# tusen-ai/SST

Hardware: AMD Instinct MI355X
Metric: LiDAR frames/sec (SST backbone fwd+bwd) at Waymo 0.32m voxels (higher is better)
Workload: dtype f32 (storage, accumulation, attention, LayerNorm, reductions: fp32; the dense products of the encoder layers from the EXACT three-way bf16 split of both fp32 operands, six bf16 MFMA products with fp32 accumulation - error vs float64 <= 2 x the fp32 matrix pipe's: tests/test_gpu_dense_f32x6.py)

## Files before the change

### sst_amd/csrc/layer_tail_x6.hip

```cpp
#include <math.h>
#include <stdlib.h>
#include "common.h"

#ifndef SST_NT_OUT
#define SST_NT_OUT false
#endif
#ifndef SST_NT_BWD
#define SST_NT_BWD true
#endif

namespace {

typedef float f32x4 __attribute__((ext_vector_type(4)));
typedef float f32x2 __attribute__((ext_vector_type(2)));
typedef unsigned u32x4 __attribute__((ext_vector_type(4)));
typedef __bf16 bf16x8 __attribute__((ext_vector_type(8)));
typedef __bf16 bf16x2 __attribute__((ext_vector_type(2)));

__device__ __forceinline__ unsigned pack2(float lo, float hi) {
  const f32x2 v = {lo, hi};
  return __builtin_bit_cast(unsigned, __builtin_convertvector(v, bf16x2));
}
__device__ __forceinline__ float lo_f(unsigned p) { return __uint_as_float(p << 16); }
__device__ __forceinline__ float hi_f(unsigned p) { return __uint_as_float(p & 0xffff0000u); }
__device__ __forceinline__ f32x4 mma32(u32x4 a, u32x4 b, f32x4 c) {
  return __builtin_amdgcn_mfma_f32_16x16x32_bf16(__builtin_bit_cast(bf16x8, a), __builtin_bit_cast(bf16x8, b), c, 0, 0, 0);
}
__device__ __forceinline__ void split2(float a, float b, unsigned& p0, unsigned& p1, unsigned& p2) {
  p0 = pack2(a, b);
  const float ra = a - lo_f(p0), rb = b - hi_f(p0);
  p1 = pack2(ra, rb);
  p2 = pack2(ra - lo_f(p1), rb - hi_f(p1));
}
struct img3 {
  u32x4 p0, p1, p2;
};
__device__ __forceinline__ img3 split8(const f32x4& a, const f32x4& b) {
  unsigned q0[4], q1[4], q2[4];
  split2(a[0], a[1], q0[0], q1[0], q2[0]);
  split2(a[2], a[3], q0[1], q1[1], q2[1]);
  split2(b[0], b[1], q0[2], q1[2], q2[2]);
  split2(b[2], b[3], q0[3], q1[3], q2[3]);
  img3 r;
  r.p0 = (u32x4){q0[0], q0[1], q0[2], q0[3]};
  r.p1 = (u32x4){q1[0], q1[1], q1[2], q1[3]};
  r.p2 = (u32x4){q2[0], q2[1], q2[2], q2[3]};
  return r;
}
__device__ __forceinline__ void join8(const img3& v, f32x4& a, f32x4& b) {
#pragma unroll
  for (int i = 0; i < 2; ++i) {
    a[2 * i] = (lo_f(v.p2[i]) + lo_f(v.p1[i])) + lo_f(v.p0[i]);
    a[2 * i + 1] = (hi_f(v.p2[i]) + hi_f(v.p1[i])) + hi_f(v.p0[i]);
    b[2 * i] = (lo_f(v.p2[2 + i]) + lo_f(v.p1[2 + i])) + lo_f(v.p0[2 + i]);
    b[2 * i + 1] = (hi_f(v.p2[2 + i]) + hi_f(v.p1[2 + i])) + hi_f(v.p0[2 + i]);
  }
}

__device__ __forceinline__ float erf_as(float z, float& e) {
  const float az = fabsf(z);
  const float t = __builtin_amdgcn_rcpf(fmaf(0.3275911f, az, 1.f));
  e = __expf(-az * az);
  const float poly = t * fmaf(t, fmaf(t, fmaf(t, fmaf(t, 1.061405429f, -1.453152027f), 1.421413741f), -0.284496736f), 0.254829592f);
  return copysignf(fmaf(-poly, e, 1.f), z);
}
__device__ __forceinline__ float gelu_f(float x) {
  float e;
  return 0.5f * x * (1.f + erf_as(x * 0.70710678118654752f, e));
}
__device__ __forceinline__ float gelu_grad_f(float x) {
  float e;
  const float phi = 0.5f * (1.f + erf_as(x * 0.70710678118654752f, e));
  return fmaf(x * 0.3989422804014327f, e, phi);
}

__device__ __forceinline__ int w_lds_row(int n) {
  const int tp = n >> 5, within = n & 31;
  return 16 * (2 * tp + ((within >> 2) & 1)) + ((within >> 3) << 2) + (within & 3);
}

template <int CTRL>
__device__ __forceinline__ float dpp_add(float v) {
  return v + __int_as_float(__builtin_amdgcn_update_dpp(0, __float_as_int(v), CTRL, 0xf, 0xf, false));
}
__device__ __forceinline__ float row_sum16(float v) {
  v = dpp_add<0xB1>(v);
  v = dpp_add<0x4E>(v);
  v = dpp_add<0x141>(v);
  return dpp_add<0x140>(v);
}

constexpr int kC = 128, kFF = 256, kHC = 32, kNF = kFF / kHC;
constexpr int kFrag = 1024;
constexpr int kI1 = 2 * 4 * kFrag;
constexpr int kI2 = 8 * 1 * kFrag;
constexpr int kIA = 8 * 2 * kFrag;
constexpr int kPart1 = 3 * kI1, kPart2 = 3 * kI2;
constexpr int kSlot = kPart1 + kPart2;
static_assert(3 * kIA <= kSlot, "slot");
#ifndef SST_TAIL_WAVES
#define SST_TAIL_WAVES 4
#endif
constexpr int kWaves = SST_TAIL_WAVES, kNTH = 64 * kWaves, kRowsPerWg = 16 * kWaves;
static_assert(kNTH >= 2 * kC, "one thread per LayerNorm parameter-gradient column");
constexpr int kNChunks = kNF + 2;
constexpr int kPackDir = kNChunks * kSlot;
constexpr int kParF = 6 * kC + kFF;
constexpr int kArea = kSlot;
constexpr int kScr = 2048;
constexpr int kLdsFwd = kArea + kParF * 4 + kWaves * kScr;
constexpr int kLdsBwd = kArea + 2 * kC * 4 + kWaves * 2 * kC * 4 + kWaves * kScr;

struct tail_weights {
  const float* wo;
  const float* w1;
  const float* w2;
};

template <bool BWD>
__device__ __forceinline__ void stage_load(const tail_weights W, int chunk, int t, float (&r)[16]) {
  if (!BWD) {
    if (chunk < 2) {
#pragma unroll
      for (int u = 0; u < 2; ++u) {
        const int idx = t + 512 * u, n = idx >> 3, k8 = (idx & 7) * 8;
        const float* p = W.wo + n * kC + 64 * chunk + k8;
        const f32x4 a = *(const f32x4*)p, b = *(const f32x4*)(p + 4);
#pragma unroll
        for (int e = 0; e < 4; ++e) r[8 * u + e] = a[e], r[8 * u + 4 + e] = b[e];
      }
    } else {
      const int j = chunk - 2;
      {
        const float* p = W.w1 + (size_t)(kHC * j + (t >> 4)) * kC + (t & 15) * 8;
        const f32x4 a = *(const f32x4*)p, b = *(const f32x4*)(p + 4);
#pragma unroll
        for (int e = 0; e < 4; ++e) r[e] = a[e], r[4 + e] = b[e];
      }
      {
        const float* p = W.w2 + (size_t)(t >> 2) * kFF + kHC * j + (t & 3) * 8;
        const f32x4 a = *(const f32x4*)p, b = *(const f32x4*)(p + 4);
#pragma unroll
        for (int e = 0; e < 4; ++e) r[8 + e] = a[e], r[12 + e] = b[e];
      }
    }
  } else {
    if (chunk >= kNF) {
      const int q = chunk - kNF;
#pragma unroll
      for (int u = 0; u < 2; ++u) {
        const int idx = t + 512 * u, jn = idx & 127, k8 = (idx >> 7) * 8;
        const float* p = W.wo + (size_t)(64 * q + k8) * kC + jn;
#pragma unroll
        for (int e = 0; e < 8; ++e) r[8 * u + e] = p[e * kC];
      }
    } else {
      const int j = chunk;
      {
        const float* p = W.w2 + (size_t)((t >> 5) * 8) * kFF + kHC * j + (t & 31);
#pragma unroll
        for (int e = 0; e < 8; ++e) r[e] = p[e * kFF];
      }
      {
        const float* p = W.w1 + (size_t)(kHC * j + (t >> 7) * 8) * kC + (t & 127);
#pragma unroll
        for (int e = 0; e < 8; ++e) r[8 + e] = p[e * kC];
      }
    }
  }
}

__device__ __forceinline__ int frag_off(int lr, int k8, int ks) {
  return ((lr >> 4) * ks + (k8 >> 5)) * kFrag + (16 * ((k8 >> 3) & 3) + (lr & 15)) * 16;
}

__device__ __forceinline__ void store_images(unsigned char* base, int image_bytes, int off, const float* v) {
  const f32x4 a = {v[0], v[1], v[2], v[3]}, b = {v[4], v[5], v[6], v[7]};
  const img3 s = split8(a, b);
  *(u32x4*)(base + off) = s.p0;
  *(u32x4*)(base + image_bytes + off) = s.p1;
  *(u32x4*)(base + 2 * image_bytes + off) = s.p2;
}

template <bool BWD>
__device__ __forceinline__ void stage_store(unsigned char* slot, int chunk, int t, const float (&r)[16]) {
  const bool outproj = BWD ? chunk >= kNF : chunk < 2;
  if (outproj) {
#pragma unroll
    for (int u = 0; u < 2; ++u) {
      const int idx = t + 512 * u;
      const int n = BWD ? (idx & 127) : (idx >> 3), k8 = BWD ? (idx >> 7) * 8 : (idx & 7) * 8;
      store_images(slot, kIA, frag_off(w_lds_row(n), k8, 2), r + 8 * u);
    }
  } else {
    const int n1 = BWD ? (t & 31) : (t >> 4), k1 = BWD ? (t >> 5) * 8 : (t & 15) * 8;
    store_images(slot, kI1, frag_off(w_lds_row(n1), k1, 4), r);
    const int n2 = BWD ? (t & 127) : (t >> 2), k2 = BWD ? (t >> 7) * 8 : (t & 3) * 8;
    store_images(slot + kPart1, kI2, frag_off(w_lds_row(n2), k2, 1), r + 8);
  }
}

constexpr int kPackMany = 16;
struct pack_batch {
  tail_weights w[kPackMany];
  unsigned char* dst[kPackMany];
};
__global__ __launch_bounds__(512) void encoder_tail_pack_k(const pack_batch B) {
  extern __shared__ __attribute__((aligned(16))) unsigned char lds[];
  const int layer = blockIdx.x / (2 * kNChunks), blk = blockIdx.x % (2 * kNChunks);
  const tail_weights W = B.w[layer];
  const int chunk = blk % kNChunks, dir = blk / kNChunks;
  float r[16];
  if (dir == 0) {
    stage_load<false>(W, chunk, threadIdx.x, r);
    stage_store<false>(lds, chunk, threadIdx.x, r);
  } else {
    stage_load<true>(W, chunk, threadIdx.x, r);
    stage_store<true>(lds, chunk, threadIdx.x, r);
  }
  __syncthreads();
  unsigned char* dst = B.dst[layer] + (size_t)blk * kSlot;
  for (int i = threadIdx.x; i < kSlot / 16; i += 512) *(u32x4*)(dst + 16 * i) = *(const u32x4*)(lds + 16 * i);
}

__device__ __forceinline__ void dma_pieces(const unsigned char* __restrict__ src, unsigned char* dst, int pieces, int wave, int lane) {
  for (int i = wave; i < pieces; i += kWaves)
    __builtin_amdgcn_global_load_lds((const __attribute__((address_space(1))) void*)(src + i * 1024 + lane * 16),
                                     (__attribute__((address_space(3))) void*)(dst + i * 1024), 16, 0, 0);
}

__device__ __forceinline__ void barrier_lds_only() { asm volatile("s_waitcnt lgkmcnt(0)\n\ts_barrier" ::: "memory"); }
__device__ __forceinline__ void barrier_drain() { asm volatile("s_waitcnt vmcnt(0) lgkmcnt(0)\n\ts_barrier" ::: "memory"); }

struct tile_io {
  unsigned char* scr;
  int frag_off0;
  int row_off[2];
  int64_t rrow[2];
  bool rvalid[2];
  int rcol;
};
__device__ __forceinline__ tile_io make_tile_io(unsigned char* scr, int lane, int64_t r0, int64_t m) {
  tile_io t;
  const int c = lane & 15, g = lane >> 4;
  t.scr = scr;
  t.frag_off0 = c * 128 + (((2 * g) ^ (c & 7)) << 4);
#pragma unroll
  for (int i = 0; i < 2; ++i) {
    const int r = 8 * i + (lane >> 3), p = lane & 7;
    t.row_off[i] = r * 128 + ((p ^ (r & 7)) << 4);
    t.rvalid[i] = r0 + r < m;
    t.rrow[i] = t.rvalid[i] ? r0 + r : m - 1;
  }
  t.rcol = (lane & 7) * 4;
  return t;
}
template <bool STREAM>
__device__ __forceinline__ void store32(const tile_io& t, float* __restrict__ base, int64_t ld, int col0, const f32x4& v0,
                                        const f32x4& v1) {
  *(f32x4*)(t.scr + t.frag_off0) = v0;
  *(f32x4*)(t.scr + (t.frag_off0 ^ 16)) = v1;
#pragma unroll
  for (int i = 0; i < 2; ++i) {
    const f32x4 w = *(const f32x4*)(t.scr + t.row_off[i]);
    if (t.rvalid[i]) {
      if (STREAM)
        __builtin_nontemporal_store(w, (f32x4*)(base + t.rrow[i] * ld + col0 + t.rcol));
      else
        *(f32x4*)(base + t.rrow[i] * ld + col0 + t.rcol) = w;
    }
  }
}
__device__ __forceinline__ void load32_issue(const tile_io& t, const float* __restrict__ base, int64_t ld, int col0, f32x4 (&w)[2]) {
#pragma unroll
  for (int i = 0; i < 2; ++i) w[i] = *(const f32x4*)(base + t.rrow[i] * ld + col0 + t.rcol);
}
__device__ __forceinline__ void load32_finish(const tile_io& t, const f32x4 (&w)[2], f32x4& v0, f32x4& v1) {
#pragma unroll
  for (int i = 0; i < 2; ++i) *(f32x4*)(t.scr + t.row_off[i]) = w[i];
  v0 = *(const f32x4*)(t.scr + t.frag_off0);
  v1 = *(const f32x4*)(t.scr + (t.frag_off0 ^ 16));
}

template <int HALF>
__device__ __forceinline__ void mma_half(const unsigned char* slot, int lane_off, const f32x4 (&x)[4][2], f32x4 (&acc)[8]) {
#pragma unroll
  for (int s2 = 0; s2 < 2; ++s2) {
    const img3 xs = split8(x[2 * HALF + s2][0], x[2 * HALF + s2][1]);
#pragma unroll
    for (int t0 = 0; t0 < 8; t0 += 4) {
      u32x4 a0[4], a1[4], a2[4];
#pragma unroll
      for (int u = 0; u < 4; ++u) {
        const int off = lane_off + ((t0 + u) * 2 + s2) * kFrag;
        a0[u] = *(const u32x4*)(slot + off);
        a1[u] = *(const u32x4*)(slot + kIA + off);
        a2[u] = *(const u32x4*)(slot + 2 * kIA + off);
      }
#pragma unroll
      for (int u = 0; u < 4; ++u) acc[t0 + u] = mma32(a0[u], xs.p2, acc[t0 + u]);
#pragma unroll
      for (int u = 0; u < 4; ++u) acc[t0 + u] = mma32(a2[u], xs.p0, acc[t0 + u]);
#pragma unroll
      for (int u = 0; u < 4; ++u) acc[t0 + u] = mma32(a1[u], xs.p1, acc[t0 + u]);
#pragma unroll
      for (int u = 0; u < 4; ++u) acc[t0 + u] = mma32(a0[u], xs.p1, acc[t0 + u]);
#pragma unroll
      for (int u = 0; u < 4; ++u) acc[t0 + u] = mma32(a1[u], xs.p0, acc[t0 + u]);
#pragma unroll
      for (int u = 0; u < 4; ++u) acc[t0 + u] = mma32(a0[u], xs.p0, acc[t0 + u]);
    }
  }
}

__device__ __forceinline__ void mma_first(const unsigned char* slot, int lane_off1, const img3 (&y)[4], f32x4& out0, f32x4& out1) {
  const f32x4 z = {0.f, 0.f, 0.f, 0.f};
  f32x4 am[2] = {z, z}, ca[2] = {z, z}, cb[2] = {z, z};
#pragma unroll
  for (int s = 0; s < 4; ++s) {
    u32x4 a0[2], a1[2], a2[2];
#pragma unroll
    for (int T = 0; T < 2; ++T) {
      const int off = lane_off1 + (T * 4 + s) * kFrag;
      a0[T] = *(const u32x4*)(slot + off);
      a1[T] = *(const u32x4*)(slot + kI1 + off);
      a2[T] = *(const u32x4*)(slot + 2 * kI1 + off);
    }
#pragma unroll
    for (int T = 0; T < 2; ++T) ca[T] = mma32(a0[T], y[s].p2, ca[T]);
#pragma unroll
    for (int T = 0; T < 2; ++T) cb[T] = mma32(a0[T], y[s].p1, cb[T]);
#pragma unroll
    for (int T = 0; T < 2; ++T) ca[T] = mma32(a2[T], y[s].p0, ca[T]);
#pragma unroll
    for (int T = 0; T < 2; ++T) am[T] = mma32(a0[T], y[s].p0, am[T]);
#pragma unroll
    for (int T = 0; T < 2; ++T) ca[T] = mma32(a1[T], y[s].p1, ca[T]);
#pragma unroll
    for (int T = 0; T < 2; ++T) cb[T] = mma32(a1[T], y[s].p0, cb[T]);
  }
  out0 = am[0] + (cb[0] + ca[0]);
  out1 = am[1] + (cb[1] + ca[1]);
}

__device__ __forceinline__ void mma_second(const unsigned char* slot2, int lane_off2, const img3& h, f32x4 (&acc)[8]) {
#pragma unroll
  for (int t0 = 0; t0 < 8; t0 += 4) {
    u32x4 a0[4], a1[4], a2[4];
#pragma unroll
    for (int u = 0; u < 4; ++u) {
      const int off = lane_off2 + (t0 + u) * kFrag;
      a0[u] = *(const u32x4*)(slot2 + off);
      a1[u] = *(const u32x4*)(slot2 + kI2 + off);
      a2[u] = *(const u32x4*)(slot2 + 2 * kI2 + off);
    }
#pragma unroll
    for (int u = 0; u < 4; ++u) acc[t0 + u] = mma32(a0[u], h.p2, acc[t0 + u]);
#pragma unroll
    for (int u = 0; u < 4; ++u) acc[t0 + u] = mma32(a2[u], h.p0, acc[t0 + u]);
#pragma unroll
    for (int u = 0; u < 4; ++u) acc[t0 + u] = mma32(a1[u], h.p1, acc[t0 + u]);
#pragma unroll
    for (int u = 0; u < 4; ++u) acc[t0 + u] = mma32(a0[u], h.p1, acc[t0 + u]);
#pragma unroll
    for (int u = 0; u < 4; ++u) acc[t0 + u] = mma32(a1[u], h.p0, acc[t0 + u]);
#pragma unroll
    for (int u = 0; u < 4; ++u) acc[t0 + u] = mma32(a0[u], h.p0, acc[t0 + u]);
  }
}

__device__ __forceinline__ void ln_stats(f32x4 (&v)[4][2], float eps, float& mean, float& rstd) {
  float sum = 0.f;
#pragma unroll
  for (int s = 0; s < 4; ++s)
#pragma unroll
    for (int r = 0; r < 4; ++r) sum += v[s][0][r] + v[s][1][r];
  sum += __shfl_xor(sum, 16, 64);
  sum += __shfl_xor(sum, 32, 64);
  mean = sum * (1.f / 128.f);
  float sq = 0.f;
#pragma unroll
  for (int s = 0; s < 4; ++s)
#pragma unroll
    for (int h = 0; h < 2; ++h)
#pragma unroll
      for (int r = 0; r < 4; ++r) {
        v[s][h][r] -= mean;
        sq = fmaf(v[s][h][r], v[s][h][r], sq);
      }
  sq += __shfl_xor(sq, 16, 64);
  sq += __shfl_xor(sq, 32, 64);
  rstd = rsqrtf(sq * (1.f / 128.f) + eps);
}

struct tail_fwd_params {
  const float *o, *x;
  const unsigned char* packed;
  const float *b_out, *b1, *b2, *n1w, *n1b, *n2w, *n2b;
  float eps;
  int64_t m;
  float *s1, *st1, *y1, *pre, *h, *s2, *st2, *y2;
  const float* pos_table;
  const int32_t* pos_idx;
  float* y2p;
};

template <int ACT>
__global__ __launch_bounds__(kNTH, 2) void encoder_tail_fwd_x6_k(const tail_fwd_params P) {
  extern __shared__ __attribute__((aligned(16))) unsigned char lds[];
  float* par = (float*)(lds + kArea);
  const int lane = threadIdx.x & 63, g = lane >> 4, c = lane & 15, wave = threadIdx.x >> 6;
  const int64_t r0 = (int64_t)blockIdx.x * kRowsPerWg + wave * 16;
  const bool valid = r0 + c < P.m;
  const int64_t row = valid ? r0 + c : P.m - 1;
  const tile_io io = make_tile_io(lds + kArea + kParF * 4 + wave * kScr, lane, r0, P.m);
  const unsigned char* packed = P.packed;
  unsigned char* const part2 = lds + kPart1;
  dma_pieces(packed, lds, 3 * kIA / 1024, wave, lane);
  f32x4 ob[4][2], xr[4][2];
  {
    f32x4 wo[4][2], wx[4][2];
#pragma unroll
    for (int s = 0; s < 4; ++s) load32_issue(io, P.o, kC, 32 * s, wo[s]);
#pragma unroll
    for (int s = 0; s < 4; ++s) load32_issue(io, P.x, kC, 32 * s, wx[s]);
#pragma unroll
    for (int s = 0; s < 4; ++s) load32_finish(io, wo[s], ob[s][0], ob[s][1]);
#pragma unroll
    for (int s = 0; s < 4; ++s) load32_finish(io, wx[s], xr[s][0], xr[s][1]);
  }
  for (int i = threadIdx.x; i < kC; i += kNTH) {
    par[i] = P.b_out ? P.b_out[i] : 0.f;
    par[kC + i] = P.n1w[i];
    par[2 * kC + i] = P.n1b[i];
    par[3 * kC + i] = P.b2 ? P.b2[i] : 0.f;
    par[4 * kC + i] = P.n2w[i];
    par[5 * kC + i] = P.n2b[i];
  }
  for (int i = threadIdx.x; i < kFF; i += kNTH) par[6 * kC + i] = P.b1 ? P.b1[i] : 0.f;

  const int lane_offA = lane * 16, lane_off1 = lane * 16, lane_off2 = lane * 16;
  const f32x4 z4 = {0.f, 0.f, 0.f, 0.f};
  f32x4 acc[8];
#pragma unroll
  for (int T = 0; T < 8; ++T) acc[T] = z4;
  img3 yi[4];

  barrier_drain();
  mma_half<0>(lds, lane_offA, ob, acc);
  barrier_drain();
  dma_pieces(packed + kSlot, lds, 3 * kIA / 1024, wave, lane);
  barrier_drain();
  mma_half<1>(lds, lane_offA, ob, acc);
  barrier_drain();
  dma_pieces(packed + 2 * kSlot, lds, kSlot / 1024, wave, lane);
  {
    f32x4 v[4][2];
#pragma unroll
    for (int s = 0; s < 4; ++s) {
      const int n0 = 32 * s + 8 * g;
      v[s][0] = acc[2 * s] + *(const f32x4*)(par + n0) + xr[s][0];
      v[s][1] = acc[2 * s + 1] + *(const f32x4*)(par + n0 + 4) + xr[s][1];
      if (P.s1 != nullptr) store32<true>(io, P.s1, kC, 32 * s, v[s][0], v[s][1]);
    }
    float mean, rstd;
    ln_stats(v, P.eps, mean, rstd);
    if (valid && g == 0) ((float2*)P.st1)[row] = make_float2(mean, rstd);
#pragma unroll
    for (int s = 0; s < 4; ++s) {
      const int n0 = 32 * s + 8 * g;
      const f32x4 y0 = v[s][0] * rstd * *(const f32x4*)(par + kC + n0) + *(const f32x4*)(par + 2 * kC + n0);
      const f32x4 y1 = v[s][1] * rstd * *(const f32x4*)(par + kC + n0 + 4) + *(const f32x4*)(par + 2 * kC + n0 + 4);
      store32<true>(io, P.y1, kC, 32 * s, y0, y1);
      yi[s] = split8(y0, y1);
    }
#pragma unroll
    for (int T = 0; T < 8; ++T) acc[T] = z4;
  }
  barrier_drain();
  f32x4 sp0 = z4, sp1 = z4, sh0 = z4, sh1 = z4;
#pragma unroll 1
  for (int j = 0; j < kNF; ++j) {
    if (j > 0) {
      store32<true>(io, P.pre, kFF, kHC * (j - 1), sp0, sp1);
      store32<true>(io, P.h, kFF, kHC * (j - 1), sh0, sh1);
    }
    f32x4 p0, p1;
    mma_first(lds, lane_off1, yi, p0, p1);
    const int nl = kHC * j + 8 * g;
    p0 += *(const f32x4*)(par + 6 * kC + nl);
    p1 += *(const f32x4*)(par + 6 * kC + nl + 4);
    f32x4 h0, h1;
#pragma unroll
    for (int r = 0; r < 4; ++r) {
      h0[r] = ACT == 1 ? gelu_f(p0[r]) : fmaxf(p0[r], 0.f);
      h1[r] = ACT == 1 ? gelu_f(p1[r]) : fmaxf(p1[r], 0.f);
    }
    const img3 hs = split8(h0, h1);
    barrier_drain();
    if (j + 1 < kNF) dma_pieces(packed + (size_t)(j + 3) * kSlot, lds, kPart1 / 1024, wave, lane);
    mma_second(part2, lane_off2, hs, acc);
    sp0 = p0, sp1 = p1, sh0 = h0, sh1 = h1;
    barrier_drain();
    if (j + 1 < kNF) dma_pieces(packed + (size_t)(j + 3) * kSlot + kPart1, part2, kPart2 / 1024, wave, lane);
  }
  store32<true>(io, P.pre, kFF, kHC * (kNF - 1), sp0, sp1);
  store32<true>(io, P.h, kFF, kHC * (kNF - 1), sh0, sh1);
  f32x4 v[4][2];
#pragma unroll
  for (int s = 0; s < 4; ++s) {
    const int n0 = 32 * s + 8 * g;
    f32x4 ya, yb;
    join8(yi[s], ya, yb);
    v[s][0] = acc[2 * s] + *(const f32x4*)(par + 3 * kC + n0) + ya;
    v[s][1] = acc[2 * s + 1] + *(const f32x4*)(par + 3 * kC + n0 + 4) + yb;
    if (P.s2 != nullptr) store32<true>(io, P.s2, kC, 32 * s, v[s][0], v[s][1]);
  }
  float mean, rstd;
  ln_stats(v, P.eps, mean, rstd);
  if (valid && g == 0) ((float2*)P.st2)[row] = make_float2(mean, rstd);
  const float* prow = P.pos_table != nullptr ? P.pos_table + (size_t)P.pos_idx[row] * kC : nullptr;
#pragma unroll
  for (int s = 0; s < 4; ++s) {
    const int n0 = 32 * s + 8 * g;
    const f32x4 y0 = v[s][0] * rstd * *(const f32x4*)(par + 4 * kC + n0) + *(const f32x4*)(par + 5 * kC + n0);
    const f32x4 y1 = v[s][1] * rstd * *(const f32x4*)(par + 4 * kC + n0 + 4) + *(const f32x4*)(par + 5 * kC + n0 + 4);
    store32<SST_NT_OUT>(io, P.y2, kC, 32 * s, y0, y1);
    if (prow != nullptr) store32<SST_NT_OUT>(io, P.y2p, kC, 32 * s, y0 + *(const f32x4*)(prow + n0), y1 + *(const f32x4*)(prow + n0 + 4));
  }
}

struct tail_bwd_params {
  const float *dy2, *dy2p, *s2, *st2, *n2w, *pre, *s1, *st1, *n1w;
  const unsigned char* packed;
  int64_t m;
  float *ds2, *dpre, *ds1, *d_o;
  float *part2, *part1;
};

__device__ __forceinline__ void ln_bwd(f32x4 (&d)[4][2], f32x4 (&sv)[4][2], const float2 st, const float* gamma, int g, int c,
                                       bool valid, float* red) {
  float sg = 0.f, sgx = 0.f;
#pragma unroll
  for (int s = 0; s < 4; ++s)
#pragma unroll
    for (int h = 0; h < 2; ++h) {
      const f32x4 w = *(const f32x4*)(gamma + 32 * s + 8 * g + 4 * h);
      sv[s][h] = (sv[s][h] - st.x) * st.y;
      f32x4 a, b;
#pragma unroll
      for (int r = 0; r < 4; ++r) {
        a[r] = row_sum16(valid ? d[s][h][r] * sv[s][h][r] : 0.f);
        b[r] = row_sum16(valid ? d[s][h][r] : 0.f);
      }
      if (c == 0) {
        *(f32x4*)(red + 32 * s + 8 * g + 4 * h) = a;
        *(f32x4*)(red + kC + 32 * s + 8 * g + 4 * h) = b;
      }
      d[s][h] *= w;
#pragma unroll
      for (int r = 0; r < 4; ++r) {
        sg += d[s][h][r];
        sgx = fmaf(d[s][h][r], sv[s][h][r], sgx);
      }
    }
  sg += __shfl_xor(sg, 16, 64);
  sg += __shfl_xor(sg, 32, 64);
  sgx += __shfl_xor(sgx, 16, 64);
  sgx += __shfl_xor(sgx, 32, 64);
  const float mg = sg * (1.f / 128.f), mgx = sgx * (1.f / 128.f);
#pragma unroll
  for (int s = 0; s < 4; ++s)
#pragma unroll
    for (int h = 0; h < 2; ++h)
#pragma unroll
      for (int r = 0; r < 4; ++r) d[s][h][r] = st.y * (d[s][h][r] - mg - sv[s][h][r] * mgx);
}

template <int ACT>
__global__ __launch_bounds__(kNTH, 2) void encoder_tail_bwd_x6_k(const tail_bwd_params P) {
  extern __shared__ __attribute__((aligned(16))) unsigned char lds[];
  float* par = (float*)(lds + kArea);
  float* red = par + 2 * kC;
  const int lane = threadIdx.x & 63, g = lane >> 4, c = lane & 15, wave = threadIdx.x >> 6;
  const int64_t r0 = (int64_t)blockIdx.x * kRowsPerWg + wave * 16;
  const bool valid = r0 + c < P.m;
  const int64_t row = valid ? r0 + c : P.m - 1;
  const tile_io io = make_tile_io(lds + kArea + 2 * kC * 4 + kWaves * 2 * kC * 4 + wave * kScr, lane, r0, P.m);
  const unsigned char* packed = P.packed;
  unsigned char* const part2 = lds + kPart1;
  dma_pieces(packed, lds, kSlot / 1024, wave, lane);
  f32x4 d[4][2], sv[4][2];
  {
    f32x4 wd[4][2], we[4][2];
#pragma unroll
    for (int s = 0; s < 4; ++s) load32_issue(io, P.dy2, kC, 32 * s, wd[s]);
    if (P.dy2p != nullptr) {
#pragma unroll
      for (int s = 0; s < 4; ++s) load32_issue(io, P.dy2p, kC, 32 * s, we[s]);
#pragma unroll
      for (int s = 0; s < 4; ++s) {
        wd[s][0] += we[s][0];
        wd[s][1] += we[s][1];
      }
    }
#pragma unroll
    for (int s = 0; s < 4; ++s) load32_issue(io, P.s2, kC, 32 * s, we[s]);
#pragma unroll
    for (int s = 0; s < 4; ++s) load32_finish(io, wd[s], d[s][0], d[s][1]);
#pragma unroll
    for (int s = 0; s < 4; ++s) load32_finish(io, we[s], sv[s][0], sv[s][1]);
  }
  const float2 st2 = ((const float2*)P.st2)[row];
  for (int i = threadIdx.x; i < kC; i += kNTH) {
    par[i] = P.n2w[i];
    par[kC + i] = P.n1w[i];
  }
  barrier_drain();

  img3 di[4];
  {
    ln_bwd(d, sv, st2, par, g, c, valid, red + wave * 2 * kC);
#pragma unroll
    for (int s = 0; s < 4; ++s) {
      store32<SST_NT_BWD>(io, P.ds2, kC, 32 * s, d[s][0], d[s][1]);
      di[s] = split8(d[s][0], d[s][1]);
    }
  }
  const int lane_offA = lane * 16, lane_off1 = lane * 16, lane_off2 = lane * 16;
  const f32x4 z4 = {0.f, 0.f, 0.f, 0.f};
  f32x4 acc[8];
#pragma unroll
  for (int T = 0; T < 8; ++T) acc[T] = z4;
  f32x4 xs1[4][2];
  f32x4 pq[2];
  load32_issue(io, P.pre, kFF, 0, pq);

  f32x4 sd0 = z4, sd1 = z4;
  auto ffn_chunk = [&](int j, const f32x4 q0, const f32x4 q1) __attribute__((always_inline)) {
    if (j > 0) store32<SST_NT_BWD>(io, P.dpre, kFF, kHC * (j - 1), sd0, sd1);
    f32x4 p0, p1;
    mma_first(lds, lane_off1, di, p0, p1);
#pragma unroll
    for (int r = 0; r < 4; ++r) {
      p0[r] *= ACT == 1 ? gelu_grad_f(q0[r]) : (q0[r] > 0.f ? 1.f : 0.f);
      p1[r] *= ACT == 1 ? gelu_grad_f(q1[r]) : (q1[r] > 0.f ? 1.f : 0.f);
    }
    const img3 hs = split8(p0, p1);
    barrier_drain();
    if (j + 1 < kNF) dma_pieces(packed + (size_t)(j + 1) * kSlot, lds, kPart1 / 1024, wave, lane);
    mma_second(part2, lane_off2, hs, acc);
    sd0 = p0, sd1 = p1;
    barrier_drain();
    if (j + 1 < kNF)
      dma_pieces(packed + (size_t)(j + 1) * kSlot + kPart1, part2, kPart2 / 1024, wave, lane);
    else
      dma_pieces(packed + (size_t)kNF * kSlot, lds, 3 * kIA / 1024, wave, lane);
  };
  barrier_drain();
  if (threadIdx.x < 2 * kC) {
    float a = 0.f;
#pragma unroll
    for (int w = 0; w < kWaves; ++w) a += red[w * 2 * kC + threadIdx.x];
    P.part2[(int64_t)blockIdx.x * 2 * kC + threadIdx.x] = a;
  }
#pragma unroll 1
  for (int j = 0; j < kNF - 1; ++j) {
    f32x4 q0, q1;
    load32_finish(io, pq, q0, q1);
    load32_issue(io, P.pre, kFF, kHC * (j + 1), pq);
    ffn_chunk(j, q0, q1);
  }
  {
    f32x4 q0, q1;
    load32_finish(io, pq, q0, q1);
    ffn_chunk(kNF - 1, q0, q1);
    store32<SST_NT_BWD>(io, P.dpre, kFF, kHC * (kNF - 1), sd0, sd1);
    {
      f32x4 ws[4][2];
#pragma unroll
      for (int s = 0; s < 4; ++s) load32_issue(io, P.s1, kC, 32 * s, ws[s]);
#pragma unroll
      for (int s = 0; s < 4; ++s) load32_finish(io, ws[s], xs1[s][0], xs1[s][1]);
    }
    f32x4 dd[4][2];
#pragma unroll
    for (int s = 0; s < 4; ++s) {
      f32x4 ya, yb;
      join8(di[s], ya, yb);
      dd[s][0] = acc[2 * s] + ya;
      dd[s][1] = acc[2 * s + 1] + yb;
    }
    const float2 st1 = ((const float2*)P.st1)[row];
    barrier_drain();
    ln_bwd(dd, xs1, st1, par + kC, g, c, valid, red + wave * 2 * kC);
#pragma unroll
    for (int s = 0; s < 4; ++s) {
      store32<SST_NT_BWD>(io, P.ds1, kC, 32 * s, dd[s][0], dd[s][1]);
      xs1[s][0] = dd[s][0];
      xs1[s][1] = dd[s][1];
    }
#pragma unroll
    for (int T = 0; T < 8; ++T) acc[T] = z4;
    barrier_drain();
    mma_half<0>(lds, lane_offA, xs1, acc);
    barrier_drain();
    dma_pieces(packed + (size_t)(kNF + 1) * kSlot, lds, 3 * kIA / 1024, wave, lane);
    barrier_drain();
    mma_half<1>(lds, lane_offA, xs1, acc);
  }
#pragma unroll
  for (int s = 0; s < 4; ++s) store32<SST_NT_OUT>(io, P.d_o, kC, 32 * s, acc[2 * s], acc[2 * s + 1]);
  barrier_drain();
  if (threadIdx.x < 2 * kC) {
    float b = 0.f;
#pragma unroll
    for (int w = 0; w < kWaves; ++w) b += red[w * 2 * kC + threadIdx.x];
    P.part1[(int64_t)blockIdx.x * 2 * kC + threadIdx.x] = b;
  }
}

bool aligned16(const void* p) { return ((uintptr_t)p & 15) == 0; }

template <typename K>
int configure(K kernel, int lds_bytes, unsigned long long* mask) {
  if (sst_first_use_on_device(mask)) {
    SST_HIP(hipFuncSetAttribute((const void*)kernel, hipFuncAttributeMaxDynamicSharedMemorySize, lds_bytes));
    sst_mark_device(mask);
  }
  return SST_OK;
}

}

int sst_internal_encoder_tail_bwd_f32x6(const sst_encoder_tail_bwd_args* a, float** part2, float** part1, int* partial_rows,
                                        void* stream) {
  if (!a || a->m <= 0 || (a->act != 1 && a->act != 2)) return SST_ERR_ARG;
  const void* need[] = {a->dy2, a->s2, a->st2, a->n2w, a->pre, a->s1, a->st1, a->n1w, a->packed,
                        a->ds2, a->dpre, a->ds1, a->d_o, a->workspace};
  for (const void* p : need)
    if (!p || !aligned16(p)) return SST_ERR_ARG;
  if (a->dy2p && !aligned16(a->dy2p)) return SST_ERR_ARG;
  const int64_t rows = sst_div_up(a->m, (int64_t)kRowsPerWg);
  if (rows > 0x7fffffff / 2) return SST_ERR_UNSUPPORTED;
  tail_bwd_params P;
  P.dy2 = a->dy2, P.dy2p = a->dy2p, P.s2 = a->s2, P.st2 = a->st2, P.n2w = a->n2w, P.pre = a->pre, P.s1 = a->s1, P.st1 = a->st1;
  P.n1w = a->n1w, P.packed = (const unsigned char*)a->packed + kPackDir, P.m = a->m;
  P.ds2 = a->ds2, P.dpre = a->dpre, P.ds1 = a->ds1, P.d_o = a->d_o;
  P.part2 = (float*)a->workspace;
  P.part1 = P.part2 + rows * 2 * kC;
  hipStream_t st = (hipStream_t)stream;
  static unsigned long long cfg1 = 0, cfg2 = 0;
  if (a->act == 1) {
    const int rc = configure(encoder_tail_bwd_x6_k<1>, kLdsBwd, &cfg1);
    if (rc) return rc;
    hipLaunchKernelGGL(encoder_tail_bwd_x6_k<1>, dim3((unsigned)rows), dim3(kNTH), kLdsBwd, st, P);
  } else {
    const int rc = configure(encoder_tail_bwd_x6_k<2>, kLdsBwd, &cfg2);
    if (rc) return rc;
    hipLaunchKernelGGL(encoder_tail_bwd_x6_k<2>, dim3((unsigned)rows), dim3(kNTH), kLdsBwd, st, P);
  }
  SST_LAUNCH_CHECK();
  *part2 = P.part2, *part1 = P.part1, *partial_rows = (int)rows;
  return SST_OK;
}

namespace {
__global__ __launch_bounds__(1024) void tail_colsum_k(const float* __restrict__ partials, int nb, int width, float* __restrict__ out0,
                                                      float* __restrict__ out1, int split) {
  __shared__ float red[32][33];
  const int cx = threadIdx.x & 31, gy = threadIdx.x >> 5;
  const int i = blockIdx.x * 32 + cx;
  float acc = 0.f;
  if (i < width)
    for (int b = gy; b < nb; b += 32) acc += partials[(int64_t)b * width + i];
  red[gy][cx] = acc;
  __syncthreads();
  if (gy == 0 && i < width) {
    float t = 0.f;
#pragma unroll
    for (int k = 0; k < 32; ++k) t += red[k][cx];
    if (i < split)
      out0[i] = t;
    else
      out1[i - split] = t;
  }
}
}

extern "C" {

int64_t sst_encoder_tail_pack_bytes(void) { return 2 * (int64_t)kPackDir; }

int sst_encoder_tail_pack_f32x6_many(const float* const* d_w_out, const float* const* d_w1, const float* const* d_w2,
                                     void* const* d_packed, int n, void* stream) {
  if (n < 0 || (n > 0 && (!d_w_out || !d_w1 || !d_w2 || !d_packed))) return SST_ERR_ARG;
  static unsigned long long cfg = 0;
  const int rc = configure(encoder_tail_pack_k, kSlot, &cfg);
  if (rc) return rc;
  for (int base = 0; base < n; base += kPackMany) {
    pack_batch B;
    const int cnt = n - base < kPackMany ? n - base : kPackMany;
    for (int i = 0; i < cnt; ++i) {
      const float *wo = d_w_out[base + i], *w1 = d_w1[base + i], *w2 = d_w2[base + i];
      void* dst = d_packed[base + i];
      if (!wo || !w1 || !w2 || !dst || !aligned16(wo) || !aligned16(w1) || !aligned16(w2) || !aligned16(dst)) return SST_ERR_ARG;
      B.w[i].wo = wo, B.w[i].w1 = w1, B.w[i].w2 = w2;
      B.dst[i] = (unsigned char*)dst;
    }
    hipLaunchKernelGGL(encoder_tail_pack_k, dim3(cnt * 2 * kNChunks), dim3(512), kSlot, (hipStream_t)stream, B);
  }
  SST_LAUNCH_CHECK();
  return SST_OK;
}

int sst_encoder_tail_pack_f32x6(const float* d_w_out, const float* d_w1, const float* d_w2, void* d_packed, void* stream) {
  return sst_encoder_tail_pack_f32x6_many(&d_w_out, &d_w1, &d_w2, &d_packed, 1, stream);
}

int64_t sst_encoder_tail_bwd_workspace_bytes(int64_t m) {
  if (m < 0) return SST_ERR_ARG;
  return sst_align_up(2 * sst_div_up(m > 0 ? m : 1, (int64_t)kRowsPerWg) * 2 * kC * (int64_t)sizeof(float), 256);
}

int sst_encoder_tail_fwd_f32x6(const sst_encoder_tail_fwd_args* a, void* stream) {
  if (!a || a->m < 0 || (a->act != 1 && a->act != 2)) return SST_ERR_ARG;
  if (a->m == 0) return SST_OK;
  const void* need[] = {a->o, a->x, a->packed, a->n1w, a->n1b, a->n2w, a->n2b, a->st1, a->y1, a->pre, a->h, a->st2, a->y2};
  for (const void* p : need)
    if (!p || !aligned16(p)) return SST_ERR_ARG;
  if ((a->s1 && !aligned16(a->s1)) || (a->s2 && !aligned16(a->s2))) return SST_ERR_ARG;
  if ((a->pos_table != nullptr) != (a->pos_idx != nullptr) || (a->pos_table != nullptr) != (a->y2p != nullptr)) return SST_ERR_ARG;
  if (a->pos_table && (!aligned16(a->pos_table) || !aligned16(a->y2p))) return SST_ERR_ARG;
  tail_fwd_params P;
  P.o = a->o, P.x = a->x, P.packed = (const unsigned char*)a->packed;
  P.b_out = a->b_out, P.b1 = a->b1, P.b2 = a->b2, P.n1w = a->n1w, P.n1b = a->n1b, P.n2w = a->n2w, P.n2b = a->n2b;
  P.eps = a->eps, P.m = a->m;
  P.s1 = a->s1, P.st1 = a->st1, P.y1 = a->y1, P.pre = a->pre, P.h = a->h, P.s2 = a->s2, P.st2 = a->st2, P.y2 = a->y2;
  P.pos_table = a->pos_table, P.pos_idx = a->pos_idx, P.y2p = a->y2p;
  const int64_t rows = sst_div_up(a->m, (int64_t)kRowsPerWg);
  if (rows > 0x7fffffff) return SST_ERR_UNSUPPORTED;
  hipStream_t st = (hipStream_t)stream;
  static unsigned long long cfg1 = 0, cfg2 = 0;
  if (a->act == 1) {
    const int rc = configure(encoder_tail_fwd_x6_k<1>, kLdsFwd, &cfg1);
    if (rc) return rc;
    hipLaunchKernelGGL(encoder_tail_fwd_x6_k<1>, dim3((unsigned)rows), dim3(kNTH), kLdsFwd, st, P);
  } else {
    const int rc = configure(encoder_tail_fwd_x6_k<2>, kLdsFwd, &cfg2);
    if (rc) return rc;
    hipLaunchKernelGGL(encoder_tail_fwd_x6_k<2>, dim3((unsigned)rows), dim3(kNTH), kLdsFwd, st, P);
  }
  SST_LAUNCH_CHECK();
  return SST_OK;
}

int sst_encoder_tail_bwd_f32x6(const sst_encoder_tail_bwd_args* a, void* stream) {
  if (!a || a->m < 0) return SST_ERR_ARG;
  if (!a->dn2w || !a->dn2b || !a->dn1w || !a->dn1b) return SST_ERR_ARG;
  hipStream_t st = (hipStream_t)stream;
  if (a->m == 0) {
    for (float* p : {a->dn2w, a->dn2b, a->dn1w, a->dn1b}) SST_HIP(hipMemsetAsync(p, 0, sizeof(float) * kC, st));
    return SST_OK;
  }
  float *part2 = nullptr, *part1 = nullptr;
  int rows = 0;
  const int rc = sst_internal_encoder_tail_bwd_f32x6(a, &part2, &part1, &rows, stream);
  if (rc) return rc;
  hipLaunchKernelGGL(tail_colsum_k, dim3(2 * kC / 32), dim3(1024), 0, st, part2, rows, 2 * kC, a->dn2w, a->dn2b, kC);
  hipLaunchKernelGGL(tail_colsum_k, dim3(2 * kC / 32), dim3(1024), 0, st, part1, rows, 2 * kC, a->dn1w, a->dn1b, kC);
  SST_LAUNCH_CHECK();
  return SST_OK;
}

}
```

Baseline: 97.05.

## Use counted vmcnt barriers and interleave global stores with FFN chunk DMA

Replaces full vmcnt drains with counted waits (barrier_keep) in both encoder tail kernels so that outstanding global stores and prefetch loads need not retire at every barrier. Per-chunk pre/h/dpre stores move inside the loop after the next DMA is issued, and the backward pass prefetches pre two chunks ahead. It also unrolls the DMA issue loops with compile-time counts, computes row addresses as 32-bit offsets from a scalar base, and skips row-validity checks for full blocks. An env var restores full drains; the counted vmcnt values depend on the exact instruction ordering and could become unsafe if the compiler reorders memory ops.

After: 97.64, median of 6. Within noise of the previous version (+0.6%).

```diff
diff --git a/sst_amd/csrc/layer_tail_x6.hip b/sst_amd/csrc/layer_tail_x6.hip
--- a/sst_amd/csrc/layer_tail_x6.hip
+++ b/sst_amd/csrc/layer_tail_x6.hip
@@ -47,7 +47,9 @@
   r.p2 = (u32x4){q2[0], q2[1], q2[2], q2[3]};
   return r;
 }
-__device__ __forceinline__ void join8(const img3& v, f32x4& a, f32x4& b) {
+__device__ __forceinline__ void join8(const img3& in, f32x4& a, f32x4& b) {
+  img3 v = in;
+  asm("" : "+v"(v.p0), "+v"(v.p1), "+v"(v.p2));
 #pragma unroll
   for (int i = 0; i < 2; ++i) {
     a[2 * i] = (lo_f(v.p2[i]) + lo_f(v.p1[i])) + lo_f(v.p0[i]);
@@ -223,20 +225,34 @@
   for (int i = threadIdx.x; i < kSlot / 16; i += 512) *(u32x4*)(dst + 16 * i) = *(const u32x4*)(lds + 16 * i);
 }
 
-__device__ __forceinline__ void dma_pieces(const unsigned char* __restrict__ src, unsigned char* dst, int pieces, int wave, int lane) {
-  for (int i = wave; i < pieces; i += kWaves)
+template <int PIECES>
+__device__ __forceinline__ void dma_pieces(const unsigned char* __restrict__ src, unsigned char* dst, int wave, int lane) {
+  static_assert(PIECES % kWaves == 0, "every wave issues the same number of pieces");
+#pragma unroll
+  for (int u = 0; u < PIECES / kWaves; ++u) {
+    const int i = wave + u * kWaves;
     __builtin_amdgcn_global_load_lds((const __attribute__((address_space(1))) void*)(src + i * 1024 + lane * 16),
                                      (__attribute__((address_space(3))) void*)(dst + i * 1024), 16, 0, 0);
+  }
 }
 
 __device__ __forceinline__ void barrier_lds_only() { asm volatile("s_waitcnt lgkmcnt(0)\n\ts_barrier" ::: "memory"); }
 __device__ __forceinline__ void barrier_drain() { asm volatile("s_waitcnt vmcnt(0) lgkmcnt(0)\n\ts_barrier" ::: "memory"); }
+template <int N>
+__device__ __forceinline__ void barrier_keep(bool counted) {
+  static_assert(N > 0 && N < 64, "vmcnt is a 6-bit field");
+  if (counted)
+    asm volatile("s_waitcnt vmcnt(%0) lgkmcnt(0)\n\ts_barrier" ::"n"(N) : "memory");
+  else
+    barrier_drain();
+}
 
 struct tile_io {
   unsigned char* scr;
   int frag_off0;
   int row_off[2];
-  int64_t rrow[2];
+  int64_t rbase;
+  int rl[2];
   bool rvalid[2];
   int rcol;
 };
@@ -245,35 +261,45 @@
   const int c = lane & 15, g = lane >> 4;
   t.scr = scr;
   t.frag_off0 = c * 128 + (((2 * g) ^ (c & 7)) << 4);
+  t.rbase = r0 < m ? r0 : m - 1;
+  const int last = (int)(m - 1 - t.rbase < 15 ? m - 1 - t.rbase : 15);
 #pragma unroll
   for (int i = 0; i < 2; ++i) {
     const int r = 8 * i + (lane >> 3), p = lane & 7;
     t.row_off[i] = r * 128 + ((p ^ (r & 7)) << 4);
     t.rvalid[i] = r0 + r < m;
-    t.rrow[i] = t.rvalid[i] ? r0 + r : m - 1;
+    t.rl[i] = r < last ? r : last;
   }
   t.rcol = (lane & 7) * 4;
   return t;
 }
+template <typename T>
+__device__ __forceinline__ T* row_addr(const tile_io& t, T* base, int ld, int col0, int i) {
+  T* const ub = base + t.rbase * ld + col0;
+  unsigned off = (unsigned)(t.rl[i] * ld + t.rcol) * (unsigned)sizeof(float);
+  asm volatile("" : "+v"(off));
+  return (T*)((const unsigned char*)ub + off);
+}
 template <bool STREAM>
-__device__ __forceinline__ void store32(const tile_io& t, float* __restrict__ base, int64_t ld, int col0, const f32x4& v0,
+__device__ __forceinline__ void store32(const tile_io& t, bool all, float* __restrict__ base, int ld, int col0, const f32x4& v0,
                                         const f32x4& v1) {
   *(f32x4*)(t.scr + t.frag_off0) = v0;
   *(f32x4*)(t.scr + (t.frag_off0 ^ 16)) = v1;
 #pragma unroll
   for (int i = 0; i < 2; ++i) {
     const f32x4 w = *(const f32x4*)(t.scr + t.row_off[i]);
-    if (t.rvalid[i]) {
+    if (all || t.rvalid[i]) {
+      f32x4* const dst = (f32x4*)row_addr(t, base, ld, col0, i);
       if (STREAM)
-        __builtin_nontemporal_store(w, (f32x4*)(base + t.rrow[i] * ld + col0 + t.rcol));
+        __builtin_nontemporal_store(w, dst);
       else
-        *(f32x4*)(base + t.rrow[i] * ld + col0 + t.rcol) = w;
-    }
-  }
-}
-__device__ __forceinline__ void load32_issue(const tile_io& t, const float* __restrict__ base, int64_t ld, int col0, f32x4 (&w)[2]) {
-#pragma unroll
-  for (int i = 0; i < 2; ++i) w[i] = *(const f32x4*)(base + t.rrow[i] * ld + col0 + t.rcol);
+        *dst = w;
+    }
+  }
+}
+__device__ __forceinline__ void load32_issue(const tile_io& t, const float* __restrict__ base, int ld, int col0, f32x4 (&w)[2]) {
+#pragma unroll
+  for (int i = 0; i < 2; ++i) w[i] = *(const f32x4*)row_addr(t, base, ld, col0, i);
 }
 __device__ __forceinline__ void load32_finish(const tile_io& t, const f32x4 (&w)[2], f32x4& v0, f32x4& v1) {
 #pragma unroll
@@ -403,20 +429,22 @@
   const float* pos_table;
   const int32_t* pos_idx;
   float* y2p;
+  int drain;
 };
 
 template <int ACT>
 __global__ __launch_bounds__(kNTH, 2) void encoder_tail_fwd_x6_k(const tail_fwd_params P) {
   extern __shared__ __attribute__((aligned(16))) unsigned char lds[];
+  const bool counted = !P.drain && (int64_t)(blockIdx.x + 1) * kRowsPerWg <= P.m;
   float* par = (float*)(lds + kArea);
-  const int lane = threadIdx.x & 63, g = lane >> 4, c = lane & 15, wave = threadIdx.x >> 6;
+  const int lane = threadIdx.x & 63, g = lane >> 4, c = lane & 15, wave = __builtin_amdgcn_readfirstlane(threadIdx.x >> 6);
   const int64_t r0 = (int64_t)blockIdx.x * kRowsPerWg + wave * 16;
   const bool valid = r0 + c < P.m;
   const int64_t row = valid ? r0 + c : P.m - 1;
   const tile_io io = make_tile_io(lds + kArea + kParF * 4 + wave * kScr, lane, r0, P.m);
   const unsigned char* packed = P.packed;
   unsigned char* const part2 = lds + kPart1;
-  dma_pieces(packed, lds, 3 * kIA / 1024, wave, lane);
+  dma_pieces<3 * kIA / 1024>(packed, lds, wave, lane);
   f32x4 ob[4][2], xr[4][2];
   {
     f32x4 wo[4][2], wx[4][2];
@@ -449,11 +477,11 @@
   barrier_drain();
   mma_half<0>(lds, lane_offA, ob, acc);
   barrier_drain();
-  dma_pieces(packed + kSlot, lds, 3 * kIA / 1024, wave, lane);
+  dma_pieces<3 * kIA / 1024>(packed + kSlot, lds, wave, lane);
   barrier_drain();
   mma_half<1>(lds, lane_offA, ob, acc);
   barrier_drain();
-  dma_pieces(packed + 2 * kSlot, lds, kSlot / 1024, wave, lane);
+  dma_pieces<kSlot / 1024>(packed + 2 * kSlot, lds, wave, lane);
   {
     f32x4 v[4][2];
 #pragma unroll
@@ -461,7 +489,7 @@
       const int n0 = 32 * s + 8 * g;
       v[s][0] = acc[2 * s] + *(const f32x4*)(par + n0) + xr[s][0];
       v[s][1] = acc[2 * s + 1] + *(const f32x4*)(par + n0 + 4) + xr[s][1];
-      if (P.s1 != nullptr) store32<true>(io, P.s1, kC, 32 * s, v[s][0], v[s][1]);
+      if (P.s1 != nullptr) store32<true>(io, counted, P.s1, kC, 32 * s, v[s][0], v[s][1]);
     }
     float mean, rstd;
     ln_stats(v, P.eps, mean, rstd);
@@ -471,20 +499,15 @@
       const int n0 = 32 * s + 8 * g;
       const f32x4 y0 = v[s][0] * rstd * *(const f32x4*)(par + kC + n0) + *(const f32x4*)(par + 2 * kC + n0);
       const f32x4 y1 = v[s][1] * rstd * *(const f32x4*)(par + kC + n0 + 4) + *(const f32x4*)(par + 2 * kC + n0 + 4);
-      store32<true>(io, P.y1, kC, 32 * s, y0, y1);
+      store32<true>(io, counted, P.y1, kC, 32 * s, y0, y1);
       yi[s] = split8(y0, y1);
     }
 #pragma unroll
     for (int T = 0; T < 8; ++T) acc[T] = z4;
   }
-  barrier_drain();
-  f32x4 sp0 = z4, sp1 = z4, sh0 = z4, sh1 = z4;
+  barrier_keep<8>(counted);
 #pragma unroll 1
   for (int j = 0; j < kNF; ++j) {
-    if (j > 0) {
-      store32<true>(io, P.pre, kFF, kHC * (j - 1), sp0, sp1);
-      store32<true>(io, P.h, kFF, kHC * (j - 1), sh0, sh1);
-    }
     f32x4 p0, p1;
     mma_first(lds, lane_off1, yi, p0, p1);
     const int nl = kHC * j + 8 * g;
@@ -497,15 +520,14 @@
       h1[r] = ACT == 1 ? gelu_f(p1[r]) : fmaxf(p1[r], 0.f);
     }
     const img3 hs = split8(h0, h1);
-    barrier_drain();
-    if (j + 1 < kNF) dma_pieces(packed + (size_t)(j + 3) * kSlot, lds, kPart1 / 1024, wave, lane);
+    barrier_keep<2>(counted);
+    if (j + 1 < kNF) dma_pieces<kPart1 / 1024>(packed + (size_t)(j + 3) * kSlot, lds, wave, lane);
+    store32<true>(io, counted, P.pre, kFF, kHC * j, p0, p1);
     mma_second(part2, lane_off2, hs, acc);
-    sp0 = p0, sp1 = p1, sh0 = h0, sh1 = h1;
-    barrier_drain();
-    if (j + 1 < kNF) dma_pieces(packed + (size_t)(j + 3) * kSlot + kPart1, part2, kPart2 / 1024, wave, lane);
-  }
-  store32<true>(io, P.pre, kFF, kHC * (kNF - 1), sp0, sp1);
-  store32<true>(io, P.h, kFF, kHC * (kNF - 1), sh0, sh1);
+    barrier_keep<2>(counted);
+    if (j + 1 < kNF) dma_pieces<kPart2 / 1024>(packed + (size_t)(j + 3) * kSlot + kPart1, part2, wave, lane);
+    store32<true>(io, counted, P.h, kFF, kHC * j, h0, h1);
+  }
   f32x4 v[4][2];
 #pragma unroll
   for (int s = 0; s < 4; ++s) {
@@ -514,7 +536,7 @@
     join8(yi[s], ya, yb);
     v[s][0] = acc[2 * s] + *(const f32x4*)(par + 3 * kC + n0) + ya;
     v[s][1] = acc[2 * s + 1] + *(const f32x4*)(par + 3 * kC + n0 + 4) + yb;
-    if (P.s2 != nullptr) store32<true>(io, P.s2, kC, 32 * s, v[s][0], v[s][1]);
+    if (P.s2 != nullptr) store32<true>(io, counted, P.s2, kC, 32 * s, v[s][0], v[s][1]);
   }
   float mean, rstd;
   ln_stats(v, P.eps, mean, rstd);
@@ -525,8 +547,9 @@
     const int n0 = 32 * s + 8 * g;
     const f32x4 y0 = v[s][0] * rstd * *(const f32x4*)(par + 4 * kC + n0) + *(const f32x4*)(par + 5 * kC + n0);
     const f32x4 y1 = v[s][1] * rstd * *(const f32x4*)(par + 4 * kC + n0 + 4) + *(const f32x4*)(par + 5 * kC + n0 + 4);
-    store32<SST_NT_OUT>(io, P.y2, kC, 32 * s, y0, y1);
-    if (prow != nullptr) store32<SST_NT_OUT>(io, P.y2p, kC, 32 * s, y0 + *(const f32x4*)(prow + n0), y1 + *(const f32x4*)(prow + n0 + 4));
+    store32<SST_NT_OUT>(io, counted, P.y2, kC, 32 * s, y0, y1);
+    if (prow != nullptr)
+      store32<SST_NT_OUT>(io, counted, P.y2p, kC, 32 * s, y0 + *(const f32x4*)(prow + n0), y1 + *(const f32x4*)(prow + n0 + 4));
   }
 }
 
@@ -536,6 +559,7 @@
   int64_t m;
   float *ds2, *dpre, *ds1, *d_o;
   float *part2, *part1;
+  int drain;
 };
 
 __device__ __forceinline__ void ln_bwd(f32x4 (&d)[4][2], f32x4 (&sv)[4][2], const float2 st, const float* gamma, int g, int c,
@@ -580,16 +604,17 @@
 template <int ACT>
 __global__ __launch_bounds__(kNTH, 2) void encoder_tail_bwd_x6_k(const tail_bwd_params P) {
   extern __shared__ __attribute__((aligned(16))) unsigned char lds[];
+  const bool counted = !P.drain && (int64_t)(blockIdx.x + 1) * kRowsPerWg <= P.m;
   float* par = (float*)(lds + kArea);
   float* red = par + 2 * kC;
-  const int lane = threadIdx.x & 63, g = lane >> 4, c = lane & 15, wave = threadIdx.x >> 6;
+  const int lane = threadIdx.x & 63, g = lane >> 4, c = lane & 15, wave = __builtin_amdgcn_readfirstlane(threadIdx.x >> 6);
   const int64_t r0 = (int64_t)blockIdx.x * kRowsPerWg + wave * 16;
   const bool valid = r0 + c < P.m;
   const int64_t row = valid ? r0 + c : P.m - 1;
   const tile_io io = make_tile_io(lds + kArea + 2 * kC * 4 + kWaves * 2 * kC * 4 + wave * kScr, lane, r0, P.m);
   const unsigned char* packed = P.packed;
   unsigned char* const part2 = lds + kPart1;
-  dma_pieces(packed, lds, kSlot / 1024, wave, lane);
+  dma_pieces<kSlot / 1024>(packed, lds, wave, lane);
   f32x4 d[4][2], sv[4][2];
   {
     f32x4 wd[4][2], we[4][2];
@@ -623,7 +648,7 @@
     ln_bwd(d, sv, st2, par, g, c, valid, red + wave * 2 * kC);
 #pragma unroll
     for (int s = 0; s < 4; ++s) {
-      store32<SST_NT_BWD>(io, P.ds2, kC, 32 * s, d[s][0], d[s][1]);
+      store32<SST_NT_BWD>(io, counted, P.ds2, kC, 32 * s, d[s][0], d[s][1]);
       di[s] = split8(d[s][0], d[s][1]);
     }
   }
@@ -634,11 +659,10 @@
   for (int T = 0; T < 8; ++T) acc[T] = z4;
   f32x4 xs1[4][2];
   f32x4 pq[2];
+  f32x4 q0, q1;
   load32_issue(io, P.pre, kFF, 0, pq);
 
-  f32x4 sd0 = z4, sd1 = z4;
-  auto ffn_chunk = [&](int j, const f32x4 q0, const f32x4 q1) __attribute__((always_inline)) {
-    if (j > 0) store32<SST_NT_BWD>(io, P.dpre, kFF, kHC * (j - 1), sd0, sd1);
+  auto ffn_chunk = [&](int j, bool request, bool last) __attribute__((always_inline)) {
     f32x4 p0, p1;
     mma_first(lds, lane_off1, di, p0, p1);
 #pragma unroll
@@ -647,35 +671,36 @@
       p1[r] *= ACT == 1 ? gelu_grad_f(q1[r]) : (q1[r] > 0.f ? 1.f : 0.f);
     }
     const img3 hs = split8(p0, p1);
+    if (last)
+      barrier_keep<2>(counted);
+    else
+      barrier_keep<4>(counted);
+    if (!last) dma_pieces<kPart1 / 1024>(packed + (size_t)(j + 1) * kSlot, lds, wave, lane);
+    mma_second(part2, lane_off2, hs, acc);
     barrier_drain();
-    if (j + 1 < kNF) dma_pieces(packed + (size_t)(j + 1) * kSlot, lds, kPart1 / 1024, wave, lane);
-    mma_second(part2, lane_off2, hs, acc);
-    sd0 = p0, sd1 = p1;
-    barrier_drain();
-    if (j + 1 < kNF)
-      dma_pieces(packed + (size_t)(j + 1) * kSlot + kPart1, part2, kPart2 / 1024, wave, lane);
-    else
-      dma_pieces(packed + (size_t)kNF * kSlot, lds, 3 * kIA / 1024, wave, lane);
+    if (!last) {
+      load32_finish(io, pq, q0, q1);
+      dma_pieces<kPart2 / 1024>(packed + (size_t)(j + 1) * kSlot + kPart1, part2, wave, lane);
+    } else {
+      dma_pieces<3 * kIA / 1024>(packed + (size_t)kNF * kSlot, lds, wave, lane);
+    }
+    store32<SST_NT_BWD>(io, counted, P.dpre, kFF, kHC * j, p0, p1);
+    if (request) load32_issue(io, P.pre, kFF, kHC * (j + 2), pq);
   };
   barrier_drain();
+  load32_finish(io, pq, q0, q1);
   if (threadIdx.x < 2 * kC) {
     float a = 0.f;
 #pragma unroll
     for (int w = 0; w < kWaves; ++w) a += red[w * 2 * kC + threadIdx.x];
     P.part2[(int64_t)blockIdx.x * 2 * kC + threadIdx.x] = a;
   }
+  load32_issue(io, P.pre, kFF, kHC, pq);
 #pragma unroll 1
-  for (int j = 0; j < kNF - 1; ++j) {
-    f32x4 q0, q1;
-    load32_finish(io, pq, q0, q1);
-    load32_issue(io, P.pre, kFF, kHC * (j + 1), pq);
-    ffn_chunk(j, q0, q1);
-  }
+  for (int j = 0; j < kNF - 2; ++j) ffn_chunk(j, true, false);
+  ffn_chunk(kNF - 2, false, false);
   {
-    f32x4 q0, q1;
-    load32_finish(io, pq, q0, q1);
-    ffn_chunk(kNF - 1, q0, q1);
-    store32<SST_NT_BWD>(io, P.dpre, kFF, kHC * (kNF - 1), sd0, sd1);
+    ffn_chunk(kNF - 1, false, true);
     {
       f32x4 ws[4][2];
 #pragma unroll
@@ -696,22 +721,28 @@
     ln_bwd(dd, xs1, st1, par + kC, g, c, valid, red + wave * 2 * kC);
 #pragma unroll
     for (int s = 0; s < 4; ++s) {
-      store32<SST_NT_BWD>(io, P.ds1, kC, 32 * s, dd[s][0], dd[s][1]);
+      store32<SST_NT_BWD>(io, counted, P.ds1, kC, 32 * s, dd[s][0], dd[s][1]);
       xs1[s][0] = dd[s][0];
       xs1[s][1] = dd[s][1];
     }
 #pragma unroll
     for (int T = 0; T < 8; ++T) acc[T] = z4;
-    barrier_drain();
+    barrier_keep<8>(counted);
     mma_half<0>(lds, lane_offA, xs1, acc);
-    barrier_drain();
-    dma_pieces(packed + (size_t)(kNF + 1) * kSlot, lds, 3 * kIA / 1024, wave, lane);
+    if (counted)
+      barrier_lds_only();
+    else
+      barrier_drain();
+    dma_pieces<3 * kIA / 1024>(packed + (size_t)(kNF + 1) * kSlot, lds, wave, lane);
     barrier_drain();
     mma_half<1>(lds, lane_offA, xs1, acc);
   }
 #pragma unroll
-  for (int s = 0; s < 4; ++s) store32<SST_NT_OUT>(io, P.d_o, kC, 32 * s, acc[2 * s], acc[2 * s + 1]);
-  barrier_drain();
+  for (int s = 0; s < 4; ++s) store32<SST_NT_OUT>(io, counted, P.d_o, kC, 32 * s, acc[2 * s], acc[2 * s + 1]);
+  if (counted)
+    barrier_lds_only();
+  else
+    barrier_drain();
   if (threadIdx.x < 2 * kC) {
     float b = 0.f;
 #pragma unroll
@@ -721,6 +752,15 @@
 }
 
 bool aligned16(const void* p) { return ((uintptr_t)p & 15) == 0; }
+
+int tail_drain() {
+  static int drain = -1;
+  if (drain < 0) {
+    const char* e = getenv("SST_AMD_TAIL_DRAIN");
+    drain = (e != nullptr && atoi(e) != 0) ? 1 : 0;
+  }
+  return drain;
+}
 
 template <typename K>
 int configure(K kernel, int lds_bytes, unsigned long long* mask) {
@@ -749,6 +789,7 @@
   P.ds2 = a->ds2, P.dpre = a->dpre, P.ds1 = a->ds1, P.d_o = a->d_o;
   P.part2 = (float*)a->workspace;
   P.part1 = P.part2 + rows * 2 * kC;
+  P.drain = tail_drain();
   hipStream_t st = (hipStream_t)stream;
   static unsigned long long cfg1 = 0, cfg2 = 0;
   if (a->act == 1) {
@@ -838,6 +879,7 @@
   P.eps = a->eps, P.m = a->m;
   P.s1 = a->s1, P.st1 = a->st1, P.y1 = a->y1, P.pre = a->pre, P.h = a->h, P.s2 = a->s2, P.st2 = a->st2, P.y2 = a->y2;
   P.pos_table = a->pos_table, P.pos_idx = a->pos_idx, P.y2p = a->y2p;
+  P.drain = tail_drain();
   const int64_t rows = sst_div_up(a->m, (int64_t)kRowsPerWg);
   if (rows > 0x7fffffff) return SST_ERR_UNSUPPORTED;
   hipStream_t st = (hipStream_t)stream;
```
